# Z-Zheng/ever

Hardware: AMD Instinct MI355X
Metric: 512x512 tiles/sec fwd+bwd, FarSeg-R50 (higher is better)
Workload: dtype f32; 1 GPU; FarSeg ResNet-50 FPN (FarSegHead defaults, BCE+dice), 3-band 512x512, batch 16/GPU, fwd+bwd+SGD step, inputs resident in HBM; global_batch=16, parallelism=single

## Files before the change

ever_amd/_C.py:

```python
import ctypes as C
import os

_LIB_PATH = os.path.join(os.path.dirname(os.path.abspath(__file__)), 'lib', 'libever_hip.so')
_LIB_PATH = os.environ.get('EVK_LIB', _LIB_PATH)

c_void_p, c_int, c_i32, c_i64, c_u32, c_f32, c_size_t = (
    C.c_void_p, C.c_int, C.c_int32, C.c_int64, C.c_uint32, C.c_float, C.c_size_t)


class ConvDesc(C.Structure):
    _fields_ = [(n, c_i32) for n in (
        'N', 'H', 'W', 'Cin', 'Ho', 'Wo', 'Cout', 'kh', 'kw',
        'stride_h', 'stride_w', 'pad_h', 'pad_w', 'dil_h', 'dil_w')]


class SplitJob(C.Structure):
    _fields_ = [('w', c_void_p), ('out', c_void_p), ('kind', c_i32), ('arg', c_i32 * 13)]


P = c_void_p
_DP = C.POINTER(ConvDesc)
_JP = C.POINTER(SplitJob)

SIGNATURES = {
# ... 66 lines not shown
                                                 P, c_size_t, P, P]),
    'evk_bn_relu_pool_bwd': (c_int, [P, P, P, P, P, P, P, P, P, P, c_i32, c_i32, c_i32, c_i32, c_i32, P, c_size_t, P, P]),
    'evk_bn_bwd': (c_int, [P, P, P, P, P, P, P, P, P, P, P, c_i64, c_i32, c_u32, c_i32, P, c_size_t, P, P]),
    'evk_stream_fork': (c_int, [P, P]),
    'evk_streams_overlap': (c_int, [P, P, c_i32, P]),
    'evk_bn_relu_dot_fwd': (c_int, [P, P, P, P, P, c_i64, c_i32, c_i32, P]),
    'evk_bn_relu_dot_workspace_bytes': (c_size_t, [c_i64, c_i32, c_i32]),
    'evk_bn_relu_dot_bwd': (c_int, [P, P, P, P, P, P, P, P, P, P, P, P, c_i64, c_i32, c_i32, c_u32, P, c_size_t, P, P]),
    'evk_bn_finalize_parts': (c_int, [P, c_i32, c_i32, c_i64, P, P, P, P, c_f32, c_f32, P, P, P, P]),
    'evk_relation_bn_fwd': (c_int, [P, P, P, P, P, P, P, c_i32, c_i32, c_i32, P, P]),
    'evk_relation_bn_parts': (c_i32, [c_i32, c_i32]),
    'evk_relation_bn_workspace_bytes': (c_size_t, [c_i32, c_i32, c_i32]),
    'evk_relation_bn_bwd': (c_int, [P, P, P, P, P, P, P, P, P, P, P, P, c_i32, c_i32, c_i32, P, c_size_t, P]),
    'evk_bn_bwd_from_partials': (c_int, [P, P, P, P, P, P, P, c_i32, P, P, P, c_i64, c_i32, c_u32, c_i32, P, c_size_t, P, P]),
    'evk_bn_bwd_bits': (c_int, [P, P, P, P, P, P, P, P, P, P, P, c_i64, c_i32, c_u32, c_i32, P, c_size_t, P, P, P]),
    'evk_relu_fwd': (c_int, [P, P, c_i64, P]),
    'evk_relu_bwd': (c_int, [P, P, P, c_i64, P]),
    'evk_add': (c_int, [P, P, P, c_i64, P]),
    'evk_scale': (c_int, [P, c_f32, P, c_i64, P]),
    'evk_group_weight_expand': (c_int, [P, P, c_i32, c_i32, c_i32, c_i32, P]),
    'evk_group_weight_gather': (c_int, [P, P, c_i32, c_i32, c_i32, c_i32, P]),
    'evk_mul_scale': (c_int, [P, P, c_f32, P, c_i64, P]),
    'evk_gelu_fwd': (c_int, [P, P, c_i64, P]),
    'evk_gelu_bwd': (c_int, [P, P, P, c_i64, P]),
    'evk_maxpool3x3s2_fwd': (c_int, [P, P, P, c_i32, c_i32, c_i32, c_i32, P]),
    'evk_maxpool3x3s2_bwd': (c_int, [P, P, P, c_i32, c_i32, c_i32, c_i32, P]),
    'evk_upsample_nearest2x_add_fwd': (c_int, [P, P, P, c_i32, c_i32, c_i32, c_i32, P, P]),
    'evk_upsample_nearest2x_bwd': (c_int, [P, P, c_i32, c_i32, c_i32, c_i32, P]),
    'evk_subsample2_fwd': (c_int, [P, P, c_i32, c_i32, c_i32, c_i32, P]),
    'evk_subsample2_bwd': (c_int, [P, P, c_i32, c_i32, c_i32, c_i32, P]),
# ... 112 lines not shown
```

ever_amd/csrc/bn.hip:

```cpp
#include "bn_common.hpp"

namespace evk {

__global__ __launch_bounds__(256) void bn_stats_partial_kernel(const float* __restrict__ x, float* __restrict__ partial,
                                                               int64_t rows, int C, int64_t rows_per_blk, int tpc,
                                                               int rl) {
  __shared__ f32x4 red[2][256];
  const int c4 = C >> 2;
  const int tc = threadIdx.x % tpc, tr = threadIdx.x / tpc;
  const int64_t r0 = (int64_t)blockIdx.x * rows_per_blk;
  const int64_t r1 = min(rows, r0 + rows_per_blk);
  for (int cb = tc; cb < c4; cb += tpc) {
    f32x4 s = {0.f, 0.f, 0.f, 0.f}, q = {0.f, 0.f, 0.f, 0.f};
    const f32x4 pv = *reinterpret_cast<const f32x4*>(x + cb * 4);
    if (tr < rl) {
      int64_t r = r0 + tr;
      const int64_t st = rl;
      for (; r + 3 * st < r1; r += 4 * st) {
        const f32x4 v0 = *reinterpret_cast<const f32x4*>(x + r * C + cb * 4) - pv;
        const f32x4 v1 = *reinterpret_cast<const f32x4*>(x + (r + st) * C + cb * 4) - pv;
        const f32x4 v2 = *reinterpret_cast<const f32x4*>(x + (r + 2 * st) * C + cb * 4) - pv;
        const f32x4 v3 = *reinterpret_cast<const f32x4*>(x + (r + 3 * st) * C + cb * 4) - pv;
        s += (v0 + v1) + (v2 + v3);
        q += (v0 * v0 + v1 * v1) + (v2 * v2 + v3 * v3);
// ... 186 lines not shown
      if (tr == 0) {
        for (int k = 1; k < rl; ++k) {
          const f32x4 a = red[0][k * tpc + tc], b = red[1][k * tpc + tc];
          gm.x = fmaxf(gm.x, a.x); gm.y = fmaxf(gm.y, a.y); gm.z = fmaxf(gm.z, a.z); gm.w = fmaxf(gm.w, a.w);
          xm.x = fmaxf(xm.x, b.x); xm.y = fmaxf(xm.y, b.y); xm.z = fmaxf(xm.z, b.z); xm.w = fmaxf(xm.w, b.w);
        }
        float* o = pmax + (size_t)bn_blk() * 2 * C;
        *reinterpret_cast<f32x4*>(o + cb * 4) = gm;
        *reinterpret_cast<f32x4*>(o + C + cb * 4) = xm;
      }
      __syncthreads();
    }
  }
}

template <int FC = kFinCh>
__global__ __launch_bounds__(256) void bn_bwd_final_kernel(const float* __restrict__ partial, int nblk, int C,
                                                           double inv_rows, const float* __restrict__ gamma,
                                                           const float* __restrict__ invstd,
                                                           float* __restrict__ dgamma, float* __restrict__ dbeta,
                                                           float* __restrict__ coef, int train,
                                                           uint32_t* __restrict__ amax,
                                                           const float* __restrict__ pmax) {
  if (!pmax) zero_amax(amax);
  float gmax = 0.f, xmax = 0.f;
  if (pmax) {
    __shared__ float mred[4][FC];
    const int tc = threadIdx.x % FC, tl = threadIdx.x / FC;
    const int cc = bn_fin_group() * FC + tc;
    if (cc < C) {
      const float* pm = pmax + cc;
      const size_t st = (size_t)2 * C;
      int b = tl;
      for (; b + 3 * (256 / FC) < nblk; b += 4 * (256 / FC)) {
        const float g0 = pm[b * st], g1 = pm[(b + (256 / FC)) * st], g2 = pm[(b + 2 * (256 / FC)) * st],
                    g3 = pm[(b + 3 * (256 / FC)) * st];
        const float x0 = pm[b * st + C], x1 = pm[(b + (256 / FC)) * st + C], x2 = pm[(b + 2 * (256 / FC)) * st + C],
                    x3 = pm[(b + 3 * (256 / FC)) * st + C];
// ... 13 lines not shown
  double s, q;
  if (!reduce_partials<FC>(partial, nblk, C, c, s, q)) return;
  if (dbeta) dbeta[c] = (float)s;
  if (dgamma) dgamma[c] = (float)q;
  const float g = gamma ? gamma[c] : 1.f;
  const float k0 = g * invstd[c], k1 = train ? (float)(s * inv_rows) : 0.f, k2 = train ? (float)(q * inv_rows) : 0.f;
  coef[c] = k0;
  coef[C + c] = k1;
  coef[2 * C + c] = k2;
  if (pmax) {
    const float bound = fabsf(k0) * (gmax + fabsf(k1) + xmax * fabsf(k2));
    uint32_t bits = __builtin_bit_cast(uint32_t, bound);
    if (bound != bound) bits = 0x7fc00000u;
    if (bits) atomicMax(&amax[0], bits);
  }
}

template <bool PK>
__global__ __launch_bounds__(256) void bn_bwd_apply_kernel(const float* __restrict__ dy, const float* __restrict__ x,
                                                           const float* __restrict__ y, const float* __restrict__ mean,
                                                           const float* __restrict__ invstd,
                                                           const float* __restrict__ coef,
                                                           const float* __restrict__ gamma,
                                                           const float* __restrict__ beta, float* __restrict__ dx,
                                                           size_t n4, int C, int relu, uint32_t* __restrict__ amax,
                                                           const uint32_t* __restrict__ bits = nullptr) {
  const size_t base = (size_t)bn_blk() * 256;
  const size_t i = base + threadIdx.x;
  const bool valid = i < n4;
  f32x4 out = {0.f, 0.f, 0.f, 0.f};
// ... 24 lines not shown
      g = relu_mask(g, yy);
    }
    const f32x4 xh = (xv - mu) * is;
    out = k0 * (g - k1 - xh * k2);
    if constexpr (PK) {
      reinterpret_cast<u32x4*>(dx)[i] = pack_hl4(out, pk_inv);
    } else {
      reinterpret_cast<f32x4*>(dx)[i] = out;
    }
  }
  if constexpr (!PK)
    if (amax) block_absmax(out, valid, amax);
}

template <int FC, int FL>
__global__ __launch_bounds__(256) void bn_parts_final_kernel(const float* __restrict__ parts, int nparts, int C,
                                                             double rows, const float* __restrict__ gamma,
                                                             const float* __restrict__ beta,
                                                             float* __restrict__ running_mean,
                                                             float* __restrict__ running_var, float momentum, float eps,
                                                             float* __restrict__ save_mean, float* __restrict__ save_invstd,
                                                             float* __restrict__ scale_shift,
                                                             uint32_t* __restrict__ amax, int pack) {
  if (!pack) zero_amax(amax);
  float E = 0.f;
  __shared__ double red[4][FC];
  const int tc = threadIdx.x % FC, tl = threadIdx.x / FC;
  const int c = bn_fin_group() * FC + tc;
  double N = 0.0, A = 0.0, B = 0.0, piv = 0.0;
  if (c < C) {
    const size_t st = (size_t)3 * C;
    piv = (double)parts[C + c];
    const float* r = parts + c;
    int b = tl;
    for (; b + 3 * FL < nparts; b += 4 * FL) {
      const float* r0 = r + (size_t)b * st;
      const float* r1 = r0 + (size_t)FL * st;
      const float* r2 = r1 + (size_t)FL * st;
// ... 36 lines not shown
  save_invstd[c] = invstd;
  const double unbias = rows > 1.0 ? rows / (rows - 1.0) : 1.0;
  if (running_mean) running_mean[c] = (1.f - momentum) * running_mean[c] + momentum * meanf;
  if (running_var) running_var[c] = (1.f - momentum) * running_var[c] + momentum * (float)(var * unbias);
  const float g = gamma ? gamma[c] : 1.f, bb = beta ? beta[c] : 0.f;
  const float sc = g * invstd;
  scale_shift[c] = sc;
  scale_shift[C + c] = bb - meanf * sc;
  if (pack) {
    const float bound = fabsf(sc) * (E * 1.001f + fabsf((float)(piv - mean))) + fabsf(bb);
    uint32_t bits = __builtin_bit_cast(uint32_t, bound);
    if (bound != bound) bits = 0x7fc00000u;
    if (bits) atomicMax(&amax[0], bits);
  }
}


static int parts_final_lanes(int nparts) { return nparts >= 1024 ? 256 : (nparts >= 512 ? 128 : 32); }

void launch_parts_final(hipStream_t st, const float* parts, int nparts, int C, double rows, const float* gamma,
                        const float* beta, float* running_mean, float* running_var, float momentum, float eps,
                        float* save_mean, float* save_invstd, float* scale_shift, uint32_t* amax, int pack) {
  const int fl = parts_final_lanes(nparts);
#define EVK_PARTS_FINAL(FC, FL)                                                                                            \
  hipLaunchKernelGGL((bn_parts_final_kernel<FC, FL>), dim3((C + FC - 1) / FC), dim3(256), 0, st, parts, nparts, C, rows, gamma, \
                     beta, running_mean, running_var, momentum, eps, save_mean, save_invstd, scale_shift, amax, pack)
  if (fl == 256) EVK_PARTS_FINAL(1, 256);
  else if (fl == 128) EVK_PARTS_FINAL(2, 128);
  else EVK_PARTS_FINAL(8, 32);
#undef EVK_PARTS_FINAL
}

void launch_bn_bwd_final(hipStream_t st, const float* partial, int nblk, int C, int64_t rows, const float* gamma,
                         const float* invstd, float* dgamma, float* dbeta, float* coef, int train, uint32_t* amax,
                         const float* pmax) {
  hipLaunchKernelGGL(bn_bwd_final_kernel<kFinCh>, dim3((C + kFinCh - 1) / kFinCh), dim3(256), 0, st, partial, nblk, C,
                     1.0 / (double)rows, gamma, invstd, dgamma, dbeta, coef, train ? 1 : 0, amax, pmax);
}

static void launch_bn_apply(hipStream_t st, bool pack, const float* x, const float* residual, const float* scale_shift,
                            float* y, int64_t rows, int C, uint32_t flags, uint32_t* amax, uint32_t* relu_bits = nullptr) {
  const size_t n4 = (size_t)rows * C / 4;
  EVK_BN_LAUNCH_PK(bn_apply_kernel, pack, dim3(oneshot_grid(n4)), 0, st, x, residual, scale_shift, y, n4, C,
                   (flags & EVK_BN_RELU) ? 1 : 0, amax, relu_bits);
}

}

using namespace evk;

extern "C" size_t evk_bn_workspace_bytes(int64_t rows, int32_t C) {
  return rows > 0 && C > 0 ? BnWorkspace::bytes(C) : 0;
}

extern "C" int evk_bn_plan(int64_t rows, int32_t C, int32_t kind, int32_t* out) {
  EVK_REQUIRE(out, EVK_E_INVALID, "bn_plan: null pointer");
  int rc = bn_check("bn_plan", rows, C, nullptr, 0, 0);
  if (rc) return rc;
  EVK_REQUIRE(kind >= 0 && kind <= 2 && (kind == 0 || rows < 0x7fffffffLL), EVK_E_UNSUPPORTED,
              "bn_plan: rows=%lld C=%d kind=%d", (long long)rows, C, kind);
// ... 120 lines not shown
  const float* gsrc = d_residual ? d_residual : dy;
  const int relu3 = d_residual ? 0 : relu;
  EVK_BN_LAUNCH_PK(bn_bwd_apply_kernel, pack, dim3(oneshot_grid(n4)), 0, st, gsrc, x, y, save_mean, save_invstd, ws.coef, gamma,
                   beta, dx, n4, C, relu3, dx_absmax, relu_bits);
  return check_launch("bn_bwd_apply");
}

extern "C" int evk_bn_bwd(const float* dy, const float* x, const float* y, const float* gamma, const float* beta,
                          const float* save_mean, const float* save_invstd, float* dx, float* d_residual,
                          float* dgamma, float* dbeta, int64_t rows, int32_t C, uint32_t flags, int32_t train,
                          void* workspace, size_t workspace_bytes, uint32_t* dx_absmax, void* stream) {
  return evk_bn_bwd_bits(dy, x, y, gamma, beta, save_mean, save_invstd, dx, d_residual, dgamma, dbeta, rows, C, flags, train,
                         workspace, workspace_bytes, dx_absmax, nullptr, stream);
}

extern "C" int evk_bn_finalize_parts(const float* parts, int32_t nparts, int32_t C, int64_t rows, const float* gamma,
                                     const float* beta, float* running_mean, float* running_var, float momentum, float eps,
                                     float* save_mean, float* save_invstd, float* scale_shift, void* stream) {
  EVK_REQUIRE(parts && nparts > 0 && save_mean && save_invstd && scale_shift, EVK_E_INVALID, "bn_finalize_parts: null pointer");
  int rc = bn_check("bn_finalize_parts", rows, C, nullptr, 0, 0);
  if (rc) return rc;
  launch_parts_final((hipStream_t)stream, parts, nparts, C, (double)rows, gamma, beta, running_mean, running_var, momentum, eps,
                     save_mean, save_invstd, scale_shift, nullptr, 0);
  return check_launch("bn_parts_final");
}
extern "C" int evk_bn_bwd_from_partials(const float* g, const float* x, const float* gamma, const float* save_mean,
                                        const float* save_invstd, const float* partial, const float* maxima, int32_t nparts,
                                        float* dx, float* dgamma, float* dbeta, int64_t rows, int32_t C, uint32_t flags,
                                        int32_t train, void* workspace, size_t workspace_bytes, uint32_t* dx_absmax,
                                        void* stream) {
// ... 147 lines not shown
```

ever_amd/hip/_base.py:

```python
import ctypes
import os

import torch
from torch.autograd import Function
from torch.autograd.function import once_differentiable

from .. import _C
from . import timing, weight_planes
from .workspace import workspace


class HipPathError(RuntimeError):
    """Raised when the HIP path is asked to run on something it cannot (CPU tensor, wrong dtype)."""


_CONV_MATH = os.environ.get('EVK_CONV_MATH', 'f16x2')
_MATH_MODES = ('f16x2', 'bf16x3', 'f32', 'bf16')


def _planes_math():
    return _CONV_MATH in ('f16x2', 'bf16x3', 'bf16')


def _f16x2():
# ... 122 lines not shown

def _mark_packed(t, bits):
    _note_amax(t, bits)
    t._evk_packed = (t._version, t.data_ptr())
    absmax_stats['packed'] += 1
    return t


def _is_packed(t):
    hit = getattr(t, '_evk_packed', None)
    return hit is not None and hit[0] == t._version and hit[1] == t.data_ptr()


_RELU_BITS = os.environ.get('EVK_RELU_BITS', '1') != '0'
_LAZY_RES = os.environ.get('EVK_LAZY_RES', '1') != '0'
relu_bits_stats = {'forward': 0, 'lazy': 0, 'masked_dgrad': 0, 'masked_bn': 0, 'materialized': 0}


def _lazy_bits(t):
    hit = getattr(t, '_evk_relu_bits', None)
    if hit is not None and hit[0] == t._version and hit[1] == t.data_ptr():
        return hit[2]
    return None


def materialize_lazy(t):
    bits = _lazy_bits(t) if t is not None else None
    if bits is None:
        return t
    out = torch.empty_like(t)
    _C.call('evk_relu_bits_apply', t.data_ptr(), bits.data_ptr(), out.data_ptr(), t.numel(), _stream())
# ... 102 lines not shown
```

ever_amd/hip/functional.py:

```python
import sys
import types

from . import _base, streams, conv, norm, pointwise, losses, depthwise, hr, fuse, transform

__all__ = [
    'HipPathError', 'empty_nhwc', 'as_nhwc', 'is_nhwc', 'image_to_nhwc', 'conv2d', 'conv2d_fork', 'conv_transpose2d', 'batch_norm_act', 'relu',
    'max_pool3x3s2', 'upsample_nearest2x_add', 'upsample_bilinear', 'global_avg_pool', 'fs_relation',
    'mean4', 'add', 'bce_with_logits', 'dice_loss_with_logits', 'cross_entropy', 'soft_cross_entropy',
    'depthwise_conv2d', 'broadcast_hw', 'hr_fuse', 'bilinear_concat', 'd4', 'd4_mean', 'weighted_fuse', 'upsample_nearest2x',
]

_PARTS = (_base, streams, conv, norm, pointwise, losses, depthwise, hr, fuse, transform)
for _m in _PARTS:
    for _k, _v in vars(_m).items():
        if not (_k.startswith('__') and _k.endswith('__')):
            globals()[_k] = _v
del _m, _k, _v


class _Facade(types.ModuleType):
    def __setattr__(self, name, value):
        for m in _PARTS:
            if name in m.__dict__:
                m.__dict__[name] = value
        types.ModuleType.__setattr__(self, name, value)


sys.modules[__name__].__class__ = _Facade
```

ever_amd/hip/norm.py:

```python
import ctypes
import os

import torch
from torch.autograd import Function
from torch.autograd.function import once_differentiable

from .. import _C
from . import timing, weight_planes
from .workspace import workspace
from ._base import (
    HipPathError, _AMAX_HANDOFF, _LAZY_RES, _PACKED, _RELU_BITS, _amax_out, _amax_zeroed, _f16x2, _inherit_amax,
    _lazy_bits, _mark_packed, _note_amax, _ptr, _require_cuda, _stream, _timed_call, as_nhwc, empty_nhwc, materialize_lazy,
    observers_active, relu_bits_stats,
)


class _BatchNormActFn(Function):

    @staticmethod
    def forward(ctx, x, residual, weight, bias, running_mean, running_var, training, momentum, eps, relu, parts=None,
                pack_out=False, lazy_res=False):
        n, c, h, w = x.shape
        rows = n * h * w
        dev = x.device
        st = _stream()
        lib = _C.load()
        ws_bytes = lib.evk_bn_workspace_bytes(rows, c)
        ws = workspace(dev, ws_bytes)
# ... 103 lines not shown
    _AMAX_HANDOFF[0] = None
    if use_batch_stats and running_mean is not None:
        weight_planes.note_running_stats_changed()
    y = _BatchNormActFn.apply(x, residual, weight, bias, running_mean, running_var, bool(use_batch_stats),
                              0.0 if momentum is None else momentum, eps, bool(relu), parts, bool(pack_out), bool(lazy_res))
    if _AMAX_HANDOFF[0] is not None:
        abits, packed = _AMAX_HANDOFF[0]
        if packed:
            _mark_packed(y, abits)
        elif abits is not None:
            _note_amax(y, abits)
        _AMAX_HANDOFF[0] = None
    return y


class _BnReluPoolFn(Function):

    @staticmethod
    def forward(ctx, x, weight, bias, running_mean, running_var, momentum, eps, parts):
        n, c, h, w = x.shape
        ho, wo = (h - 1) // 2 + 1, (w - 1) // 2 + 1
        dev, st = x.device, _stream()
        ws_bytes = _C.load().evk_bn_workspace_bytes(n * h * w, c)
        ws = workspace(dev, ws_bytes)
        y = empty_nhwc(n, c, ho, wo, dev)
        code = torch.empty((n, ho, wo, c), device=dev, dtype=torch.uint8)
        save_mean = torch.empty((c,), device=dev, dtype=torch.float32)
        save_invstd = torch.empty((c,), device=dev, dtype=torch.float32)
        abits = _amax_out(dev)
        nb = 4.0 * x.numel() + 5.0 * y.numel()
# ... 68 lines not shown
```

ever_amd/module/_resnets.py:

```python
import torch.nn as nn

from ..hip import functional as HF
from .fold import _takes_epilogue_stats, _use_folded, conv_bn
from .layers import AdaptiveAvgPool2d, BatchNorm2d, Conv2d, GroupNorm, HipSequential, MaxPool2d, ReLU

__all__ = ['ResNet', 'BasicBlock', 'Bottleneck', 'resnet18', 'resnet34', 'resnet50', 'resnet101', 'resnet152',
           'resnext50_32x4d', 'resnext101_32x4d', 'resnext101_32x8d', 'resnet50_v1c', 'resnet101_v1c']


def conv3x3(cin, cout, stride=1, groups=1, dilation=1):
    return Conv2d(cin, cout, kernel_size=3, stride=stride, padding=dilation, groups=groups, bias=False,
                  dilation=dilation)


def conv1x1(cin, cout, stride=1):
    return Conv2d(cin, cout, kernel_size=1, stride=stride, bias=False)


def _norm(norm_layer):
    if norm_layer is None or norm_layer is nn.BatchNorm2d or norm_layer is BatchNorm2d:
        return BatchNorm2d

    def make(num_features):
        m = norm_layer(num_features)
# ... 9 lines not shown


def _plain_norm(m):
    return not isinstance(m, BatchNorm2d)


def _norm_act(norm, x, relu):
    return norm(x, relu=relu) if isinstance(norm, GroupNorm) else (HF.relu(norm(x)) if relu else norm(x))


def _inference(bn):
    import torch
    return (not bn.training) and not torch.is_grad_enabled()


def _fork(block, x):
    if block.downsample is None:
        return HF.conv2d_fork(x, block.conv1, bn_stats=(_takes_epilogue_stats(block.bn1), False))
    h, s = HF.conv2d_fork(x, block.conv1, block.downsample[0],
                          bn_stats=(_takes_epilogue_stats(block.bn1), _takes_epilogue_stats(block.downsample[1])))
    return h, block.downsample[1](s)


def _lazy_ok(block, bn):
    from .layers import BatchNorm2d
    if type(bn) is not BatchNorm2d or bn._forward_hooks:
        return False
    mods = [block.conv1]
    ds = block.downsample
    if ds is not None:
        if len(ds) != 2 or type(ds[1]) is not BatchNorm2d:
            return False
        mods += [ds, ds[0], ds[1]]
    return not any(m._forward_hooks or m._forward_pre_hooks for m in mods)


# ... 13 lines not shown
        self.relu = ReLU(inplace=True)
        self.conv2 = conv3x3(planes, planes)
        self.bn2 = norm_layer(planes)
        self.downsample = downsample
        self.stride = stride

    def forward(self, x):
        if _plain_norm(self.bn1):
            shortcut = x if self.downsample is None else self.downsample(x)
            out = _norm_act(self.bn1, self.conv1(x), True)
            return HF.relu(HF.add(_norm_act(self.bn2, self.conv2(out), False), shortcut))
        if _inference(self.bn1):
            shortcut = x if self.downsample is None else conv_bn(self.downsample[0], self.downsample[1], x)
            out = conv_bn(self.conv1, self.bn1, x, relu=True)
            return conv_bn(self.conv2, self.bn2, out, residual=shortcut, relu=True)
        h, shortcut = _fork(self, x)
        out = self.bn1(h, relu=True, conv_only=True)
        return conv_bn(self.conv2, self.bn2, out, residual=shortcut, relu=True, lazy_res=_lazy_ok(self, self.bn2))


class Bottleneck(nn.Module):
    expansion = 4

    def __init__(self, inplanes, planes, stride=1, downsample=None, groups=1, base_width=64, dilation=1,
                 norm_layer=None):
        super().__init__()
        norm_layer = _norm(norm_layer)
        width = int(planes * (base_width / 64.)) * groups
        self.conv1 = conv1x1(inplanes, width)
        self.bn1 = norm_layer(width)
        self.conv2 = conv3x3(width, width, stride, groups, dilation)
        self.bn2 = norm_layer(width)
        self.conv3 = conv1x1(width, planes * self.expansion)
# ... 1 lines not shown
        self.relu = ReLU(inplace=True)
        self.downsample = downsample
        self.stride = stride

    def forward(self, x):
        if _plain_norm(self.bn1):
            shortcut = x if self.downsample is None else self.downsample(x)
            out = _norm_act(self.bn1, self.conv1(x), True)
            out = _norm_act(self.bn2, self.conv2(out), True)
            return HF.relu(HF.add(_norm_act(self.bn3, self.conv3(out), False), shortcut))
        if _inference(self.bn1):
            shortcut = x if self.downsample is None else conv_bn(self.downsample[0], self.downsample[1], x)
            out = conv_bn(self.conv1, self.bn1, x, relu=True)
            out = conv_bn(self.conv2, self.bn2, out, relu=True)
            return conv_bn(self.conv3, self.bn3, out, residual=shortcut, relu=True)
        h, shortcut = _fork(self, x)
        out = self.bn1(h, relu=True, conv_only=True)
        out = conv_bn(self.conv2, self.bn2, out, relu=True, conv_only=True)
        return conv_bn(self.conv3, self.bn3, out, residual=shortcut, relu=True, lazy_res=_lazy_ok(self, self.bn3))


class ResNet(nn.Module):
    def __init__(self, block, layers, num_classes=1000, zero_init_residual=False, groups=1, width_per_group=64,
                 replace_stride_with_dilation=None, norm_layer=None, deep_stem=False):
        super().__init__()
        norm_layer = _norm(norm_layer)
        self._norm_layer = norm_layer
        self.inplanes = 64
        self.dilation = 1
        if replace_stride_with_dilation is None:
            replace_stride_with_dilation = [False, False, False]
        if len(replace_stride_with_dilation) != 3:
            raise ValueError('replace_stride_with_dilation should be None or a 3-element tuple, got {}'.format(
                replace_stride_with_dilation))
# ... 138 lines not shown
```

include/ever_hip.h:

```cpp
#ifndef EVER_HIP_H_
#define EVER_HIP_H_

#include <stddef.h>
#include <stdint.h>

#ifdef __cplusplus
extern "C" {
#endif

#define EVK_OK 0
#define EVK_E_INVALID (-1)
#define EVK_E_UNSUPPORTED (-2)
#define EVK_E_LAUNCH (-3)
#define EVK_E_WORKSPACE (-4)

const char* evk_last_error(void);
int evk_abi_version(void);
const char* evk_build_arch(void);

typedef struct evk_conv_desc {
  int32_t N, H, W, Cin;
  int32_t Ho, Wo, Cout;
  int32_t kh, kw;
  int32_t stride_h, stride_w;
// ... 148 lines not shown
                         size_t workspace_bytes, uint32_t* dx_absmax, void* stream);
int evk_bn_fwd_eval(const float* x, const float* residual, const float* gamma, const float* beta,
                    const float* running_mean, const float* running_var, float eps, float* y,
                    float* save_mean , float* save_invstd ,
                    int64_t rows, int32_t C, uint32_t flags, void* workspace, size_t workspace_bytes,
                    uint32_t* y_absmax, void* stream);
int evk_bn_bwd(const float* dy, const float* x, const float* y, const float* gamma, const float* beta,
               const float* save_mean, const float* save_invstd, float* dx, float* d_residual,
               float* dgamma, float* dbeta, int64_t rows, int32_t C, uint32_t flags, int32_t train,
               void* workspace, size_t workspace_bytes, uint32_t* dx_absmax, void* stream);
int evk_bn_bwd_bits(const float* dy, const float* x, const float* y, const float* gamma, const float* beta,
                    const float* save_mean, const float* save_invstd, float* dx, float* d_residual,
                    float* dgamma, float* dbeta, int64_t rows, int32_t C, uint32_t flags, int32_t train,
                    void* workspace, size_t workspace_bytes, uint32_t* dx_absmax, const uint32_t* relu_bits, void* stream);

int evk_stream_fork(void* from, void* to);

int evk_streams_overlap(void* a, void* b, int32_t us, float* elapsed_us);

int evk_relu_fwd(const float* x, float* y, int64_t n, void* stream);
int evk_relu_bwd(const float* dy, const float* y, float* dx, int64_t n, void* stream);
int evk_add(const float* a, const float* b, float* out, int64_t n, void* stream);
int evk_scale(const float* a, float alpha, float* out, int64_t n, void* stream);
int evk_group_weight_expand(const float* w, float* dense, int32_t Cout, int32_t taps, int32_t Cin, int32_t groups, void* stream);
int evk_group_weight_gather(const float* ddense, float* dw, int32_t Cout, int32_t taps, int32_t Cin, int32_t groups, void* stream);
int evk_mul_scale(const float* a, const float* b, float alpha, float* out, int64_t n, void* stream);
int evk_gelu_fwd(const float* x, float* y, int64_t n, void* stream);
int evk_gelu_bwd(const float* dy, const float* x, float* dx, int64_t n, void* stream);

int evk_maxpool3x3s2_fwd(const float* x, float* y, uint8_t* code, int32_t N, int32_t H, int32_t W,
// ... 201 lines not shown
```

Baseline: 571.9 tiles/s.

## Fuse main-branch and downsample BatchNorm into dual forward and backward kernels

Adds dual-BatchNorm kernels for the block's final conv BN and the downsample shortcut BN. The forward applies both normalisations, the residual add and ReLU in a single pass, and the backward computes both branches' partial reductions and dx in shared passes over dy. ResNet blocks with a downsample now keep the raw shortcut conv output and route through this path when the eligibility conditions hold. The goal is fewer memory passes and kernel launches at the cost of extra code paths and fallback complexity.

```diff
diff --git a/ever_amd/_C.py b/ever_amd/_C.py
--- a/ever_amd/_C.py
+++ b/ever_amd/_C.py
@@ -104,6 +104,10 @@
     'evk_relation_bn_bwd': (c_int, [P, P, P, P, P, P, P, P, P, P, P, P, c_i32, c_i32, c_i32, P, c_size_t, P]),
     'evk_bn_bwd_from_partials': (c_int, [P, P, P, P, P, P, P, c_i32, P, P, P, c_i64, c_i32, c_u32, c_i32, P, c_size_t, P, P]),
     'evk_bn_bwd_bits': (c_int, [P, P, P, P, P, P, P, P, P, P, P, c_i64, c_i32, c_u32, c_i32, P, c_size_t, P, P, P]),
+    'evk_bn_fwd_train_parts_dual': (c_int, [P, P, P, P, P, P, c_f32, c_f32, P, P, P, P, c_f32, c_f32, P, P, P, P, P, c_i64, c_i32,
+                                            P, c_i32, P, c_i32, P, c_size_t, P, P, P]),
+    'evk_bn_bwd_dual': (c_int, [P, P, P, P, P, P, P, P, P, P, P, P, P, P, P, c_i64, c_i32, c_u32, c_u32, P, c_size_t, P, P, P, P]),
+    'evk_bn_bwd_dual_fused': (c_int, [c_u32, c_u32]),
     'evk_relu_fwd': (c_int, [P, P, c_i64, P]),
     'evk_relu_bwd': (c_int, [P, P, P, c_i64, P]),
     'evk_add': (c_int, [P, P, P, c_i64, P]),
diff --git a/ever_amd/csrc/bn.hip b/ever_amd/csrc/bn.hip
--- a/ever_amd/csrc/bn.hip
+++ b/ever_amd/csrc/bn.hip
@@ -224,14 +224,14 @@
   }
 }
 
-template <int FC = kFinCh>
-__global__ __launch_bounds__(256) void bn_bwd_final_kernel(const float* __restrict__ partial, int nblk, int C,
-                                                           double inv_rows, const float* __restrict__ gamma,
-                                                           const float* __restrict__ invstd,
-                                                           float* __restrict__ dgamma, float* __restrict__ dbeta,
-                                                           float* __restrict__ coef, int train,
-                                                           uint32_t* __restrict__ amax,
-                                                           const float* __restrict__ pmax) {
+template <int FC>
+__device__ __forceinline__ void bn_bwd_final_body(const float* __restrict__ partial, int nblk, int C,
+                                                  double inv_rows, const float* __restrict__ gamma,
+                                                  const float* __restrict__ invstd,
+                                                  float* __restrict__ dgamma, float* __restrict__ dbeta,
+                                                  float* __restrict__ coef, int train,
+                                                  uint32_t* __restrict__ amax,
+                                                  const float* __restrict__ pmax) {
   if (!pmax) zero_amax(amax);
   float gmax = 0.f, xmax = 0.f;
   if (pmax) {
@@ -275,6 +275,16 @@
     if (bound != bound) bits = 0x7fc00000u;
     if (bits) atomicMax(&amax[0], bits);
   }
+}
+template <int FC = kFinCh>
+__global__ __launch_bounds__(256) void bn_bwd_final_kernel(const float* __restrict__ partial, int nblk, int C,
+                                                           double inv_rows, const float* __restrict__ gamma,
+                                                           const float* __restrict__ invstd,
+                                                           float* __restrict__ dgamma, float* __restrict__ dbeta,
+                                                           float* __restrict__ coef, int train,
+                                                           uint32_t* __restrict__ amax,
+                                                           const float* __restrict__ pmax) {
+  bn_bwd_final_body<FC>(partial, nblk, C, inv_rows, gamma, invstd, dgamma, dbeta, coef, train, amax, pmax);
 }
 
 template <bool PK>
@@ -329,14 +339,14 @@
 }
 
 template <int FC, int FL>
-__global__ __launch_bounds__(256) void bn_parts_final_kernel(const float* __restrict__ parts, int nparts, int C,
-                                                             double rows, const float* __restrict__ gamma,
-                                                             const float* __restrict__ beta,
-                                                             float* __restrict__ running_mean,
-                                                             float* __restrict__ running_var, float momentum, float eps,
-                                                             float* __restrict__ save_mean, float* __restrict__ save_invstd,
-                                                             float* __restrict__ scale_shift,
-                                                             uint32_t* __restrict__ amax, int pack) {
+__device__ __forceinline__ void bn_parts_final_body(const float* __restrict__ parts, int nparts, int C,
+                                                    double rows, const float* __restrict__ gamma,
+                                                    const float* __restrict__ beta,
+                                                    float* __restrict__ running_mean,
+                                                    float* __restrict__ running_var, float momentum, float eps,
+                                                    float* __restrict__ save_mean, float* __restrict__ save_invstd,
+                                                    float* __restrict__ scale_shift,
+                                                    uint32_t* __restrict__ amax, int pack) {
   if (!pack) zero_amax(amax);
   float E = 0.f;
   __shared__ double red[4][FC];
@@ -403,6 +413,45 @@
     if (bits) atomicMax(&amax[0], bits);
   }
 }
+template <int FC, int FL>
+__global__ __launch_bounds__(256) void bn_parts_final_kernel(const float* __restrict__ parts, int nparts, int C,
+                                                             double rows, const float* __restrict__ gamma,
+                                                             const float* __restrict__ beta,
+                                                             float* __restrict__ running_mean,
+                                                             float* __restrict__ running_var, float momentum, float eps,
+                                                             float* __restrict__ save_mean, float* __restrict__ save_invstd,
+                                                             float* __restrict__ scale_shift,
+                                                             uint32_t* __restrict__ amax, int pack) {
+  bn_parts_final_body<FC, FL>(parts, nparts, C, rows, gamma, beta, running_mean, running_var, momentum, eps, save_mean,
+                              save_invstd, scale_shift, amax, pack);
+}
+
+struct BnPartsFinalSet {
+  const float* parts;
+  int nparts;
+  const float *gamma, *beta;
+  float *running_mean, *running_var;
+  float momentum, eps;
+  float *save_mean, *save_invstd, *scale_shift;
+  uint32_t* amax;
+};
+template <int FC, int FL>
+__global__ __launch_bounds__(256) void bn_parts_final_dual_kernel(BnPartsFinalSet a, BnPartsFinalSet b, int C, double rows) {
+  const BnPartsFinalSet s = blockIdx.y ? b : a;
+  bn_parts_final_body<FC, FL>(s.parts, s.nparts, C, rows, s.gamma, s.beta, s.running_mean, s.running_var, s.momentum, s.eps,
+                              s.save_mean, s.save_invstd, s.scale_shift, s.amax, 0);
+}
+struct BnBwdFinalSet {
+  const float *partial, *gamma, *invstd;
+  float *dgamma, *dbeta, *coef;
+  uint32_t* amax;
+  const float* pmax;
+};
+__global__ __launch_bounds__(256) void bn_bwd_final_dual_kernel(BnBwdFinalSet a, BnBwdFinalSet b, int nblk, int C,
+                                                                double inv_rows) {
+  const BnBwdFinalSet s = blockIdx.y ? b : a;
+  bn_bwd_final_body<kFinCh>(s.partial, nblk, C, inv_rows, s.gamma, s.invstd, s.dgamma, s.dbeta, s.coef, 1, s.amax, s.pmax);
+}
 
 
 static int parts_final_lanes(int nparts) { return nparts >= 1024 ? 256 : (nparts >= 512 ? 128 : 32); }
@@ -433,6 +482,181 @@
   EVK_BN_LAUNCH_PK(bn_apply_kernel, pack, dim3(oneshot_grid(n4)), 0, st, x, residual, scale_shift, y, n4, C,
                    (flags & EVK_BN_RELU) ? 1 : 0, amax, relu_bits);
 }
+
+
+__global__ __launch_bounds__(256) void bn_apply_dual_kernel(const float* __restrict__ za, const float* __restrict__ zb,
+                                                            const float* __restrict__ scale_shift_a,
+                                                            const float* __restrict__ scale_shift_b, float* __restrict__ y,
+                                                            size_t n4, int C, uint32_t* __restrict__ amax,
+                                                            uint32_t* __restrict__ relu_bits) {
+  const size_t base = (size_t)bn_blk() * 256;
+  const size_t i = base + threadIdx.x;
+  const bool valid = i < n4;
+  f32x4 v = {0.f, 0.f, 0.f, 0.f};
+  if (valid) {
+    const int c4 = C >> 2;
+    const int cb = chunk_of(base, c4);
+    const f32x4 sca = reinterpret_cast<const f32x4*>(scale_shift_a)[cb];
+    const f32x4 sha = reinterpret_cast<const f32x4*>(scale_shift_a + C)[cb];
+    const f32x4 scb = reinterpret_cast<const f32x4*>(scale_shift_b)[cb];
+    const f32x4 shb = reinterpret_cast<const f32x4*>(scale_shift_b + C)[cb];
+    const f32x4 yb = bn_ld(zb, i) * scb + shb;
+    v = bn_ld(za, i) * sca + sha;
+    v += yb;
+  }
+  if (((i >> 6) << 6) < n4) relu_bits_store(relu_bits, i >> 6, v.x > 0.f, v.y > 0.f, v.z > 0.f, v.w > 0.f);
+  if (valid) {
+    v.x = fmaxf(v.x, 0.f); v.y = fmaxf(v.y, 0.f); v.z = fmaxf(v.z, 0.f); v.w = fmaxf(v.w, 0.f);
+    reinterpret_cast<f32x4*>(y)[i] = v;
+  }
+  if (amax) block_absmax(v, valid, amax);
+}
+
+template <bool PK>
+__global__ __launch_bounds__(256) void bn_bwd_partial_dual_kernel(
+    const float* __restrict__ dy, const float* __restrict__ xa, const float* __restrict__ xb,
+    const float* __restrict__ mean_a, const float* __restrict__ invstd_a, const float* __restrict__ mean_b,
+    const float* __restrict__ invstd_b, float* __restrict__ partial_a, float* __restrict__ partial_b, int64_t rows, int C,
+    int64_t rows_per_blk, int tpc, int rl, float* __restrict__ pmax_a, float* __restrict__ pmax_b,
+    const uint32_t* __restrict__ bits) {
+  __shared__ f32x4 red[2][256];
+  const int c4 = C >> 2;
+  const int tc = threadIdx.x % tpc, tr = threadIdx.x / tpc;
+  const int64_t r0 = (int64_t)bn_blk() * rows_per_blk;
+  const int64_t r1 = min(rows, r0 + rows_per_blk);
+  for (int cb = tc; cb < c4; cb += tpc) {
+    const f32x4 mua = *reinterpret_cast<const f32x4*>(mean_a + cb * 4);
+    const f32x4 isa = *reinterpret_cast<const f32x4*>(invstd_a + cb * 4);
+    const f32x4 mub = *reinterpret_cast<const f32x4*>(mean_b + cb * 4);
+    const f32x4 isb = *reinterpret_cast<const f32x4*>(invstd_b + cb * 4);
+    f32x4 s = {0.f, 0.f, 0.f, 0.f}, qa = {0.f, 0.f, 0.f, 0.f}, qb = {0.f, 0.f, 0.f, 0.f};
+    f32x4 gm = {0.f, 0.f, 0.f, 0.f}, xma = {0.f, 0.f, 0.f, 0.f}, xmb = {0.f, 0.f, 0.f, 0.f};
+    if (tr < rl) {
+      auto one = [&](const f32x4 gin, const f32x4 xva, const f32x4 xvb, size_t off) {
+        const f32x4 g = relu_bits_mask(gin, bits, off >> 2);
+        s += g;
+        const f32x4 xha = (xva - mua) * isa;
+        qa += g * xha;
+        const f32x4 xhb = (xvb - mub) * isb;
+        qb += g * xhb;
+        if constexpr (PK) {
+          gm.x = fmaxf(gm.x, fabsf(g.x)); gm.y = fmaxf(gm.y, fabsf(g.y));
+          gm.z = fmaxf(gm.z, fabsf(g.z)); gm.w = fmaxf(gm.w, fabsf(g.w));
+          xma.x = fmaxf(xma.x, fabsf(xha.x)); xma.y = fmaxf(xma.y, fabsf(xha.y));
+          xma.z = fmaxf(xma.z, fabsf(xha.z)); xma.w = fmaxf(xma.w, fabsf(xha.w));
+          xmb.x = fmaxf(xmb.x, fabsf(xhb.x)); xmb.y = fmaxf(xmb.y, fabsf(xhb.y));
+          xmb.z = fmaxf(xmb.z, fabsf(xhb.z)); xmb.w = fmaxf(xmb.w, fabsf(xhb.w));
+        }
+      };
+      int64_t r = r0 + tr;
+      const int64_t st = rl;
+      for (; r + 3 * st < r1; r += 4 * st) {
+        const size_t o0 = (size_t)r * C + cb * 4, o1 = (size_t)(r + st) * C + cb * 4;
+        const size_t o2 = (size_t)(r + 2 * st) * C + cb * 4, o3 = (size_t)(r + 3 * st) * C + cb * 4;
+        const f32x4 g0 = bp_ld(dy + o0), g1 = bp_ld(dy + o1);
+        const f32x4 g2 = bp_ld(dy + o2), g3 = bp_ld(dy + o3);
+        const f32x4 a0 = bp_ld(xa + o0), a1 = bp_ld(xa + o1);
+        const f32x4 a2 = bp_ld(xa + o2), a3 = bp_ld(xa + o3);
+        const f32x4 b0 = bp_ld(xb + o0), b1 = bp_ld(xb + o1);
+        const f32x4 b2 = bp_ld(xb + o2), b3 = bp_ld(xb + o3);
+        one(g0, a0, b0, o0);
+        one(g1, a1, b1, o1);
+        one(g2, a2, b2, o2);
+        one(g3, a3, b3, o3);
+      }
+      for (; r < r1; r += st) {
+        const size_t o0 = (size_t)r * C + cb * 4;
+        one(bp_ld(dy + o0), bp_ld(xa + o0), bp_ld(xb + o0), o0);
+      }
+    }
+    fold_store_record(red, s, qa, partial_a, bn_blk(), C, cb, tc, tr, tpc, rl);
+    fold_store_record(red, s, qb, partial_b, bn_blk(), C, cb, tc, tr, tpc, rl);
+    if constexpr (PK) {
+      red[0][threadIdx.x] = gm;
+      red[1][threadIdx.x] = xma;
+      __syncthreads();
+      if (tr == 0) {
+        for (int k = 1; k < rl; ++k) {
+          const f32x4 a = red[0][k * tpc + tc], b = red[1][k * tpc + tc];
+          gm.x = fmaxf(gm.x, a.x); gm.y = fmaxf(gm.y, a.y); gm.z = fmaxf(gm.z, a.z); gm.w = fmaxf(gm.w, a.w);
+          xma.x = fmaxf(xma.x, b.x); xma.y = fmaxf(xma.y, b.y); xma.z = fmaxf(xma.z, b.z); xma.w = fmaxf(xma.w, b.w);
+        }
+      }
+      __syncthreads();
+      red[0][threadIdx.x] = xmb;
+      __syncthreads();
+      if (tr == 0) {
+        for (int k = 1; k < rl; ++k) {
+          const f32x4 b = red[0][k * tpc + tc];
+          xmb.x = fmaxf(xmb.x, b.x); xmb.y = fmaxf(xmb.y, b.y); xmb.z = fmaxf(xmb.z, b.z); xmb.w = fmaxf(xmb.w, b.w);
+        }
+        float* oa = pmax_a + (size_t)bn_blk() * 2 * C;
+        float* ob = pmax_b + (size_t)bn_blk() * 2 * C;
+        *reinterpret_cast<f32x4*>(oa + cb * 4) = gm;
+        *reinterpret_cast<f32x4*>(oa + C + cb * 4) = xma;
+        *reinterpret_cast<f32x4*>(ob + cb * 4) = gm;
+        *reinterpret_cast<f32x4*>(ob + C + cb * 4) = xmb;
+      }
+      __syncthreads();
+    }
+  }
+}
+
+template <bool PKA, bool PKB>
+__global__ __launch_bounds__(256) void bn_bwd_apply_dual_kernel(
+    const float* __restrict__ dy, const float* __restrict__ xa, const float* __restrict__ xb,
+    const float* __restrict__ mean_a, const float* __restrict__ invstd_a, const float* __restrict__ coef_a,
+    const float* __restrict__ mean_b, const float* __restrict__ invstd_b, const float* __restrict__ coef_b,
+    float* __restrict__ dxa, float* __restrict__ dxb, size_t n4, int C, uint32_t* __restrict__ amax_a,
+    uint32_t* __restrict__ amax_b, const uint32_t* __restrict__ bits) {
+  const size_t base = (size_t)bn_blk() * 256;
+  const size_t i = base + threadIdx.x;
+  const bool valid = i < n4;
+  f32x4 outa = {0.f, 0.f, 0.f, 0.f}, outb = {0.f, 0.f, 0.f, 0.f};
+  float pk_inv_a = 1.f, pk_inv_b = 1.f;
+  if constexpr (PKA) pk_inv_a = op_scale(amax_a[0]).inv;
+  if constexpr (PKB) pk_inv_b = op_scale(amax_b[0]).inv;
+  if (valid) {
+    const int c4 = C >> 2;
+    const int c = chunk_of(base, c4);
+    const f32x4 g = relu_bits_mask(bn_ld(dy, i), bits, i);
+    {
+      const f32x4 k0 = reinterpret_cast<const f32x4*>(coef_a)[c];
+      const f32x4 k1 = reinterpret_cast<const f32x4*>(coef_a + C)[c];
+      const f32x4 k2 = reinterpret_cast<const f32x4*>(coef_a + 2 * C)[c];
+      const f32x4 mu = reinterpret_cast<const f32x4*>(mean_a)[c];
+      const f32x4 is = reinterpret_cast<const f32x4*>(invstd_a)[c];
+      const f32x4 xh = (bn_ld(xa, i) - mu) * is;
+      outa = k0 * (g - k1 - xh * k2);
+      if constexpr (PKA) {
+        reinterpret_cast<u32x4*>(dxa)[i] = pack_hl4(outa, pk_inv_a);
+      } else {
+        reinterpret_cast<f32x4*>(dxa)[i] = outa;
+      }
+    }
+    {
+      const f32x4 k0 = reinterpret_cast<const f32x4*>(coef_b)[c];
+      const f32x4 k1 = reinterpret_cast<const f32x4*>(coef_b + C)[c];
+      const f32x4 k2 = reinterpret_cast<const f32x4*>(coef_b + 2 * C)[c];
+      const f32x4 mu = reinterpret_cast<const f32x4*>(mean_b)[c];
+      const f32x4 is = reinterpret_cast<const f32x4*>(invstd_b)[c];
+      const f32x4 xh = (bn_ld(xb, i) - mu) * is;
+      outb = k0 * (g - k1 - xh * k2);
+      if constexpr (PKB) {
+        reinterpret_cast<u32x4*>(dxb)[i] = pack_hl4(outb, pk_inv_b);
+      } else {
+        reinterpret_cast<f32x4*>(dxb)[i] = outb;
+      }
+    }
+  }
+  if constexpr (!PKA)
+    if (amax_a) block_absmax(outa, valid, amax_a);
+  if constexpr (!PKA && !PKB) __syncthreads();
+  if constexpr (!PKB)
+    if (amax_b) block_absmax(outb, valid, amax_b);
+}
+
+static bool bn_dual_fused(bool pack_a, bool pack_b) { return !(pack_a && !pack_b); }
 
 }
 
@@ -583,6 +807,103 @@
                          workspace, workspace_bytes, dx_absmax, nullptr, stream);
 }
 
+extern "C" int evk_bn_fwd_train_parts_dual(const float* za, const float* zb, const float* gamma_a, const float* beta_a,
+                                           float* running_mean_a, float* running_var_a, float momentum_a, float eps_a,
+                                           const float* gamma_b, const float* beta_b, float* running_mean_b,
+                                           float* running_var_b, float momentum_b, float eps_b, float* y, float* save_mean_a,
+                                           float* save_invstd_a, float* save_mean_b, float* save_invstd_b, int64_t rows,
+                                           int32_t C, const float* parts_a, int32_t nparts_a, const float* parts_b,
+                                           int32_t nparts_b, void* workspace, size_t workspace_bytes, uint32_t* y_absmax,
+                                           uint32_t* relu_bits, void* stream) {
+  EVK_REQUIRE(za && zb && y && save_mean_a && save_invstd_a && save_mean_b && save_invstd_b && parts_a && parts_b &&
+                  nparts_a > 0 && nparts_b > 0 && relu_bits,
+              EVK_E_INVALID, "bn_fwd_train_parts_dual: bad argument");
+  int rc = bn_check("bn_fwd_train_parts_dual", rows, C, workspace, workspace_bytes, 2 * BnWorkspace::bytes(C));
+  if (rc) return rc;
+  hipStream_t st = (hipStream_t)stream;
+  float* ss_a = BnWorkspace(workspace, C).coef;
+  float* ss_b = BnWorkspace((char*)workspace + BnWorkspace::bytes(C), C).coef;
+  const int fl = parts_final_lanes(nparts_a);
+  if (fl == parts_final_lanes(nparts_b)) {
+    const BnPartsFinalSet sa = {parts_a, nparts_a, gamma_a, beta_a, running_mean_a, running_var_a, momentum_a, eps_a,
+                                save_mean_a, save_invstd_a, ss_a, y_absmax};
+    const BnPartsFinalSet sb = {parts_b, nparts_b, gamma_b, beta_b, running_mean_b, running_var_b, momentum_b, eps_b,
+                                save_mean_b, save_invstd_b, ss_b, nullptr};
+#define EVK_PARTS_FINAL_DUAL(FC, FL)                                                                                       \
+  hipLaunchKernelGGL((bn_parts_final_dual_kernel<FC, FL>), dim3((C + FC - 1) / FC, 2), dim3(256), 0, st, sa, sb, C, (double)rows)
+    if (fl == 256) EVK_PARTS_FINAL_DUAL(1, 256);
+    else if (fl == 128) EVK_PARTS_FINAL_DUAL(2, 128);
+    else EVK_PARTS_FINAL_DUAL(8, 32);
+#undef EVK_PARTS_FINAL_DUAL
+    rc = check_launch("bn_parts_final_dual");
+    if (rc) return rc;
+  } else {
+    launch_parts_final(st, parts_b, nparts_b, C, (double)rows, gamma_b, beta_b, running_mean_b, running_var_b, momentum_b,
+                       eps_b, save_mean_b, save_invstd_b, ss_b, nullptr, 0);
+    rc = check_launch("bn_parts_final");
+    if (rc) return rc;
+    launch_parts_final(st, parts_a, nparts_a, C, (double)rows, gamma_a, beta_a, running_mean_a, running_var_a, momentum_a,
+                       eps_a, save_mean_a, save_invstd_a, ss_a, y_absmax, 0);
+    rc = check_launch("bn_parts_final");
+    if (rc) return rc;
+  }
+  const size_t n4 = (size_t)rows * C / 4;
+  hipLaunchKernelGGL(bn_apply_dual_kernel, dim3(oneshot_grid(n4)), dim3(256), 0, st, za, zb, (const float*)ss_a,
+                     (const float*)ss_b, y, n4, C, y_absmax, relu_bits);
+  return check_launch("bn_apply_dual");
+}
+
+extern "C" int evk_bn_bwd_dual_fused(uint32_t flags_a, uint32_t flags_b) {
+  return bn_dual_fused((flags_a & EVK_BN_PACK_DX) != 0, (flags_b & EVK_BN_PACK_DX) != 0) ? 1 : 0;
+}
+
+extern "C" int evk_bn_bwd_dual(const float* dy, const float* za, const float* zb, const float* gamma_a,
+                               const float* save_mean_a, const float* save_invstd_a, const float* gamma_b,
+                               const float* save_mean_b, const float* save_invstd_b, float* dza, float* dzb, float* dgamma_a,
+                               float* dbeta_a, float* dgamma_b, float* dbeta_b, int64_t rows, int32_t C, uint32_t flags_a,
+                               uint32_t flags_b, void* workspace, size_t workspace_bytes, uint32_t* dza_absmax,
+                               uint32_t* dzb_absmax, const uint32_t* relu_bits, void* stream) {
+  EVK_REQUIRE(dy && za && zb && save_mean_a && save_invstd_a && save_mean_b && save_invstd_b && dza && dzb && relu_bits,
+              EVK_E_INVALID, "bn_bwd_dual: null pointer");
+  int rc = bn_check("bn_bwd_dual", rows, C, workspace, workspace_bytes, 2 * BnWorkspace::bytes(C));
+  if (rc) return rc;
+  const bool pack_a = (flags_a & EVK_BN_PACK_DX) != 0, pack_b = (flags_b & EVK_BN_PACK_DX) != 0;
+  EVK_REQUIRE((!pack_a || dza_absmax) && (!pack_b || dzb_absmax), EVK_E_INVALID,
+              "bn_bwd_dual: EVK_BN_PACK_DX needs the output's absmax buffer (slots zero on entry)");
+  if (!bn_dual_fused(pack_a, pack_b)) {
+    rc = evk_bn_bwd_bits(dy, za, nullptr, gamma_a, nullptr, save_mean_a, save_invstd_a, dza, nullptr, dgamma_a, dbeta_a, rows, C,
+                         EVK_BN_RELU | (flags_a & EVK_BN_PACK_DX), 1, workspace, workspace_bytes, dza_absmax, relu_bits, stream);
+    if (rc) return rc;
+    return evk_bn_bwd_bits(dy, zb, nullptr, gamma_b, nullptr, save_mean_b, save_invstd_b, dzb, nullptr, dgamma_b, dbeta_b, rows,
+                           C, flags_b & EVK_BN_PACK_DX, 1, workspace, workspace_bytes, dzb_absmax, relu_bits, stream);
+  }
+  hipStream_t st = (hipStream_t)stream;
+  const BnPlan pl = bn_plan(rows, C);
+  const BnWorkspace wa(workspace, C), wb((char*)workspace + BnWorkspace::bytes(C), C);
+  const bool pack = pack_a || pack_b;
+  EVK_BN_LAUNCH_PK(bn_bwd_partial_dual_kernel, pack, dim3(pl.nblk), 0, st, dy, za, zb, save_mean_a, save_invstd_a, save_mean_b,
+                   save_invstd_b, wa.partial, wb.partial, rows, C, pl.rows_per_blk, pl.tpc, pl.rl, pack ? wa.pmax : nullptr,
+                   pack ? wb.pmax : nullptr, relu_bits);
+  rc = check_launch("bn_bwd_partial_dual");
+  if (rc) return rc;
+  const BnBwdFinalSet fa = {wa.partial, gamma_a, save_invstd_a, dgamma_a, dbeta_a, wa.coef, dza_absmax, pack_a ? wa.pmax : nullptr};
+  const BnBwdFinalSet fb = {wb.partial, gamma_b, save_invstd_b, dgamma_b, dbeta_b, wb.coef, dzb_absmax, pack_b ? wb.pmax : nullptr};
+  hipLaunchKernelGGL(bn_bwd_final_dual_kernel, dim3((C + kFinCh - 1) / kFinCh, 2), dim3(256), 0, st, fa, fb, pl.nblk, C,
+                     1.0 / (double)rows);
+  rc = check_launch("bn_bwd_final_dual");
+  if (rc) return rc;
+  const size_t n4 = (size_t)rows * C / 4;
+#define EVK_BN_APPLY_DUAL(PA, PB)                                                                                            \
+  hipLaunchKernelGGL((bn_bwd_apply_dual_kernel<PA, PB>), dim3(oneshot_grid(n4)), dim3(256), 0, st, dy, za, zb, save_mean_a,    \
+                     save_invstd_a, (const float*)wa.coef, save_mean_b, save_invstd_b, (const float*)wb.coef, dza, dzb, n4, C, \
+                     dza_absmax, dzb_absmax, relu_bits)
+  if (pack_a) EVK_BN_APPLY_DUAL(true, true);
+  else if (pack_b) EVK_BN_APPLY_DUAL(false, true);
+  else EVK_BN_APPLY_DUAL(false, false);
+#undef EVK_BN_APPLY_DUAL
+  return check_launch("bn_bwd_apply_dual");
+}
+
 extern "C" int evk_bn_finalize_parts(const float* parts, int32_t nparts, int32_t C, int64_t rows, const float* gamma,
                                      const float* beta, float* running_mean, float* running_var, float momentum, float eps,
                                      float* save_mean, float* save_invstd, float* scale_shift, void* stream) {
diff --git a/ever_amd/hip/_base.py b/ever_amd/hip/_base.py
--- a/ever_amd/hip/_base.py
+++ b/ever_amd/hip/_base.py
@@ -160,7 +160,7 @@
 
 _RELU_BITS = os.environ.get('EVK_RELU_BITS', '1') != '0'
 _LAZY_RES = os.environ.get('EVK_LAZY_RES', '1') != '0'
-relu_bits_stats = {'forward': 0, 'lazy': 0, 'masked_dgrad': 0, 'masked_bn': 0, 'materialized': 0}
+relu_bits_stats = {'forward': 0, 'lazy': 0, 'masked_dgrad': 0, 'masked_bn': 0, 'materialized': 0, 'dual': 0}
 
 
 def _lazy_bits(t):
diff --git a/ever_amd/hip/functional.py b/ever_amd/hip/functional.py
--- a/ever_amd/hip/functional.py
+++ b/ever_amd/hip/functional.py
@@ -27,3 +27,9 @@
 
 
 sys.modules[__name__].__class__ = _Facade
+
+
+def set_bn_dual(on):
+    me = sys.modules[__name__]
+    prev, me._BN_DUAL = me._BN_DUAL, bool(on)
+    return prev
diff --git a/ever_amd/hip/norm.py b/ever_amd/hip/norm.py
--- a/ever_amd/hip/norm.py
+++ b/ever_amd/hip/norm.py
@@ -10,8 +10,8 @@
 from .workspace import workspace
 from ._base import (
     HipPathError, _AMAX_HANDOFF, _LAZY_RES, _PACKED, _RELU_BITS, _amax_out, _amax_zeroed, _f16x2, _inherit_amax,
-    _lazy_bits, _mark_packed, _note_amax, _ptr, _require_cuda, _stream, _timed_call, as_nhwc, empty_nhwc, materialize_lazy,
-    observers_active, relu_bits_stats,
+    _lazy_bits, _mark_packed, _note_amax, _ptr, _require_cuda, _stream, _timed_call, as_nhwc, empty_nhwc, is_nhwc,
+    materialize_lazy, observers_active, relu_bits_stats,
 )
 
 
@@ -145,6 +145,113 @@
     return y
 
 
+_BN_DUAL = os.environ.get('EVK_BN_DUAL', '1') != '0'
+
+
+def bn_dual_enabled():
+    return _BN_DUAL and _RELU_BITS and _LAZY_RES
+
+
+class _BatchNormDualFn(Function):
+
+    @staticmethod
+    def forward(ctx, za, zb, weight_a, bias_a, rm_a, rv_a, momentum_a, eps_a, weight_b, bias_b, rm_b, rv_b, momentum_b,
+                eps_b, parts_a, parts_b):
+        n, c, h, w = za.shape
+        rows = n * h * w
+        dev = za.device
+        st = _stream()
+        lib = _C.load()
+        ws_bytes = 2 * lib.evk_bn_workspace_bytes(rows, c)
+        ws = workspace(dev, ws_bytes)
+        y = empty_nhwc(n, c, h, w, dev)
+        saves = [torch.empty((c,), device=dev, dtype=torch.float32) for _ in range(4)]
+        abits = _amax_out(dev)
+        rbits = torch.empty((lib.evk_relu_bits_bytes(za.numel()) // 4,), device=dev, dtype=torch.int32)
+        relu_bits_stats['forward'] += 1
+        relu_bits_stats['dual'] += 1
+        _timed_call('bn', 4.0 * za.numel() * 3, 'evk_bn_fwd_train_parts_dual', za.data_ptr(), zb.data_ptr(), _ptr(weight_a),
+                    _ptr(bias_a), _ptr(rm_a), _ptr(rv_a), float(momentum_a), float(eps_a), _ptr(weight_b), _ptr(bias_b),
+                    _ptr(rm_b), _ptr(rv_b), float(momentum_b), float(eps_b), y.data_ptr(), saves[0].data_ptr(),
+                    saves[1].data_ptr(), saves[2].data_ptr(), saves[3].data_ptr(), rows, c, parts_a[0].data_ptr(), parts_a[1],
+                    parts_b[0].data_ptr(), parts_b[1], ws.data_ptr(), ws_bytes, _ptr(abits), rbits.data_ptr(), st)
+        _AMAX_HANDOFF[0] = (abits, False)
+        ctx.pack_dx = tuple(bool(len(p) > 2 and p[2]) for p in (parts_a, parts_b))
+        ctx.save_for_backward(za, zb, weight_a, weight_b, *saves, rbits)
+        ctx.mark_non_differentiable(*[t for t in (rm_a, rv_a, rm_b, rv_b) if t is not None])
+        return y
+
+    @staticmethod
+    @once_differentiable
+    def backward(ctx, dy):
+        za, zb, weight_a, weight_b, mean_a, invstd_a, mean_b, invstd_b, rbits = ctx.saved_tensors
+        n, c, h, w = za.shape
+        rows = n * h * w
+        dev = za.device
+        st = _stream()
+        dy = as_nhwc(materialize_lazy(dy), 'batch_norm.backward')
+        lib = _C.load()
+        ws_bytes = 2 * lib.evk_bn_workspace_bytes(rows, c)
+        ws = workspace(dev, ws_bytes)
+        dza, dzb = torch.empty_like(za), torch.empty_like(zb)
+
+        def affine_grads(weight):
+            if weight is None:
+                return None, None
+            return (torch.empty((c,), device=dev, dtype=torch.float32), torch.empty((c,), device=dev, dtype=torch.float32))
+        dgamma_a, dbeta_a = affine_grads(weight_a)
+        dgamma_b, dbeta_b = affine_grads(weight_b)
+        packs, scales = [], []
+        for want in ctx.pack_dx:
+            pack = want and _f16x2()
+            abits = _amax_zeroed(dev) if pack else _amax_out(dev)
+            packs.append(bool(pack and abits is not None))
+            scales.append(abits)
+        relu_bits_stats['lazy'] += 1
+        relu_bits_stats['masked_bn'] += 1
+        _timed_call('bn', 4.0 * za.numel() * 8, 'evk_bn_bwd_dual', dy.data_ptr(), za.data_ptr(), zb.data_ptr(), _ptr(weight_a),
+                    mean_a.data_ptr(), invstd_a.data_ptr(), _ptr(weight_b), mean_b.data_ptr(), invstd_b.data_ptr(),
+                    dza.data_ptr(), dzb.data_ptr(), _ptr(dgamma_a), _ptr(dbeta_a), _ptr(dgamma_b), _ptr(dbeta_b), rows, c,
+                    2 if packs[0] else 0, 2 if packs[1] else 0, ws.data_ptr(), ws_bytes, _ptr(scales[0]), _ptr(scales[1]),
+                    rbits.data_ptr(), st)
+        for dz, pack, abits in ((dza, packs[0], scales[0]), (dzb, packs[1], scales[1])):
+            if pack:
+                _mark_packed(dz, abits)
+            elif abits is not None:
+                _note_amax(dz, abits)
+        need = ctx.needs_input_grad
+        return (dza, dzb, dgamma_a if need[2] else None, dbeta_a if need[3] else None, None, None, None, None,
+                dgamma_b if need[8] else None, dbeta_b if need[9] else None, None, None, None, None, None, None)
+
+
+def batch_norm_act_dual(za, bn_a, zb, bn_b):
+    pa, pb = getattr(za, '_evk_bn_parts', None), getattr(zb, '_evk_bn_parts', None)
+    if (not (_BN_DUAL and _RELU_BITS and _LAZY_RES) or pa is None or pb is None or pa[1] <= 0 or pb[1] <= 0
+            or za.shape != zb.shape or za.shape[1] % 4 or not (torch.is_grad_enabled() and za.requires_grad and zb.requires_grad)
+            or not (is_nhwc(za) and is_nhwc(zb)) or observers_active()):
+        return None
+    for bn in (bn_a, bn_b):
+        if not bn.training or bn.momentum is None or za.shape[0] * za.shape[2] * za.shape[3] == 1:
+            return None
+    del za._evk_bn_parts, zb._evk_bn_parts
+    args = []
+    for bn in (bn_b, bn_a):
+        if bn.track_running_stats and bn.num_batches_tracked is not None:
+            bn._nbt_pending = getattr(bn, '_nbt_pending', 0) + 1
+        track = bn.track_running_stats
+        if track and bn.running_mean is not None:
+            weight_planes.note_running_stats_changed()
+        args.append((bn.weight, bn.bias, bn.running_mean if track else None, bn.running_var if track else None,
+                     bn.momentum, bn.eps))
+    _AMAX_HANDOFF[0] = None
+    y = _BatchNormDualFn.apply(za, zb, *args[1], *args[0], pa, pb)
+    if _AMAX_HANDOFF[0] is not None:
+        if _AMAX_HANDOFF[0][0] is not None:
+            _note_amax(y, _AMAX_HANDOFF[0][0])
+        _AMAX_HANDOFF[0] = None
+    return y
+
+
 class _BnReluPoolFn(Function):
 
     @staticmethod
diff --git a/ever_amd/module/_resnets.py b/ever_amd/module/_resnets.py
--- a/ever_amd/module/_resnets.py
+++ b/ever_amd/module/_resnets.py
@@ -47,12 +47,31 @@
     return (not bn.training) and not torch.is_grad_enabled()
 
 
-def _fork(block, x):
+def _fork(block, x, raw_shortcut=False):
     if block.downsample is None:
         return HF.conv2d_fork(x, block.conv1, bn_stats=(_takes_epilogue_stats(block.bn1), False))
     h, s = HF.conv2d_fork(x, block.conv1, block.downsample[0],
                           bn_stats=(_takes_epilogue_stats(block.bn1), _takes_epilogue_stats(block.downsample[1])))
-    return h, block.downsample[1](s)
+    return h, (s if raw_shortcut else block.downsample[1](s))
+
+
+def _dual_ok(block, conv, bn):
+    ds = block.downsample
+    if ds is None or not HF.bn_dual_enabled() or not _lazy_ok(block, bn) or _use_folded(conv, bn):
+        return False
+    if not (_takes_epilogue_stats(bn) and _takes_epilogue_stats(ds[1]) and bn.training and ds[1].training):
+        return False
+    return not any(m._backward_hooks or m._backward_pre_hooks or m._forward_pre_hooks for m in (bn, ds[1]))
+
+
+def _block_end(block, conv, bn, out, s, dual):
+    if dual:
+        z = conv(out, bn_stats=True)
+        y = HF.batch_norm_act_dual(z, bn, s, block.downsample[1])
+        if y is not None:
+            return y
+        return bn(z, residual=block.downsample[1](s), relu=True, lazy_res=True)
+    return conv_bn(conv, bn, out, residual=s, relu=True, lazy_res=_lazy_ok(block, bn))
 
 
 def _lazy_ok(block, bn):
@@ -96,9 +115,10 @@
             shortcut = x if self.downsample is None else conv_bn(self.downsample[0], self.downsample[1], x)
             out = conv_bn(self.conv1, self.bn1, x, relu=True)
             return conv_bn(self.conv2, self.bn2, out, residual=shortcut, relu=True)
-        h, shortcut = _fork(self, x)
+        dual = _dual_ok(self, self.conv2, self.bn2)
+        h, shortcut = _fork(self, x, raw_shortcut=dual)
         out = self.bn1(h, relu=True, conv_only=True)
-        return conv_bn(self.conv2, self.bn2, out, residual=shortcut, relu=True, lazy_res=_lazy_ok(self, self.bn2))
+        return _block_end(self, self.conv2, self.bn2, out, shortcut, dual)
 
 
 class Bottleneck(nn.Module):
@@ -130,10 +150,11 @@
             out = conv_bn(self.conv1, self.bn1, x, relu=True)
             out = conv_bn(self.conv2, self.bn2, out, relu=True)
             return conv_bn(self.conv3, self.bn3, out, residual=shortcut, relu=True)
-        h, shortcut = _fork(self, x)
+        dual = _dual_ok(self, self.conv3, self.bn3)
+        h, shortcut = _fork(self, x, raw_shortcut=dual)
         out = self.bn1(h, relu=True, conv_only=True)
         out = conv_bn(self.conv2, self.bn2, out, relu=True, conv_only=True)
-        return conv_bn(self.conv3, self.bn3, out, residual=shortcut, relu=True, lazy_res=_lazy_ok(self, self.bn3))
+        return _block_end(self, self.conv3, self.bn3, out, shortcut, dual)
 
 
 class ResNet(nn.Module):
diff --git a/include/ever_hip.h b/include/ever_hip.h
--- a/include/ever_hip.h
+++ b/include/ever_hip.h
@@ -186,6 +186,20 @@
                     float* dgamma, float* dbeta, int64_t rows, int32_t C, uint32_t flags, int32_t train,
                     void* workspace, size_t workspace_bytes, uint32_t* dx_absmax, const uint32_t* relu_bits, void* stream);
 
+int evk_bn_fwd_train_parts_dual(const float* za, const float* zb, const float* gamma_a, const float* beta_a,
+                                float* running_mean_a, float* running_var_a, float momentum_a, float eps_a,
+                                const float* gamma_b, const float* beta_b, float* running_mean_b, float* running_var_b,
+                                float momentum_b, float eps_b, float* y, float* save_mean_a, float* save_invstd_a,
+                                float* save_mean_b, float* save_invstd_b, int64_t rows, int32_t C, const float* parts_a,
+                                int32_t nparts_a, const float* parts_b, int32_t nparts_b, void* workspace,
+                                size_t workspace_bytes, uint32_t* y_absmax, uint32_t* relu_bits, void* stream);
+int evk_bn_bwd_dual(const float* dy, const float* za, const float* zb, const float* gamma_a, const float* save_mean_a,
+                    const float* save_invstd_a, const float* gamma_b, const float* save_mean_b, const float* save_invstd_b,
+                    float* dza, float* dzb, float* dgamma_a, float* dbeta_a, float* dgamma_b, float* dbeta_b, int64_t rows,
+                    int32_t C, uint32_t flags_a, uint32_t flags_b, void* workspace, size_t workspace_bytes,
+                    uint32_t* dza_absmax, uint32_t* dzb_absmax, const uint32_t* relu_bits, void* stream);
+int evk_bn_bwd_dual_fused(uint32_t flags_a, uint32_t flags_b);
+
 int evk_stream_fork(void* from, void* to);
 
 int evk_streams_overlap(void* a, void* b, int32_t us, float* elapsed_us);
```

Measured after the change: 580.3 tiles/s, median of 6. +1.5%, better.
